# zubair-irshad/NeO-360

Hardware: NVIDIA H100
Metric: rays/sec at 640x480, 192 samples/ray (higher is better)
Workload: dtype f16 operands, f32 accumulate (wgmma)

## Files before the change

### neo360_b200/csrc/field_tc.cu

```cuda
#include "common.cuh"
#include "hopper.cuh"
#include <cuda.h>
#include <cuda_fp16.h>
#include <cstdio>
#include <cstring>

namespace neo {
namespace tc {
using namespace hopper;

constexpr int kTileRays = 32;
constexpr int kTileSamples = 2;
constexpr int kTilePts = kTileRays * kTileSamples;
constexpr int kConsumers = 2;
constexpr int kThreads = 128 * (kConsumers + 1);
constexpr int kLaunchRegs = 65536 / kThreads / 8 * 8;
constexpr int kConsumerRegs = 224, kProducerRegs = 56;
static_assert(kConsumers * 128 * kConsumerRegs + 128 * kProducerRegs == kThreads * kLaunchRegs, "setmaxnreg split must fill the CTA's registers");
static_assert(kConsumers * kTilePts == 128, "the producer warpgroup has one thread per point of each consumer's tile");

constexpr uint32_t WH_H = 0, WH_DIR = 20480, WH_V1 = 30720, WH_RGB = 38912, WH_BYTES = 40960;
constexpr int BIAS_FLOATS = 512 + 64 + 64 + 4 + 4;
constexpr uint32_t BIAS_BYTES = 2624;
constexpr uint32_t SLAB = 128 * 128;

__host__ __device__ constexpr int enc_slabs(int KE) { return (KE + 63) / 64; }
__host__ __device__ constexpr uint32_t trunk_off(int KE, int seg) { return seg == 0 ? 0u : (uint32_t)(enc_slabs(KE) + 2 * (seg - 1)) * SLAB; }
__host__ __device__ constexpr uint32_t trunk_bytes(int KE) { return trunk_off(KE, 4) + (uint32_t)(KE / 64) * SLAB; }
__host__ __device__ constexpr uint32_t w3enc_tail(int KE) { return trunk_off(KE, 0) + (uint32_t)(KE / 64) * SLAB; }
__host__ __device__ constexpr uint32_t w3enc_kstep(int KE, int ks) {
    return ks < 4 * (KE / 64) ? trunk_off(KE, 4) + (uint32_t)(ks >> 2) * SLAB + (uint32_t)(ks & 3) * 32u
                              : w3enc_tail(KE) + (uint32_t)(ks - 4 * (KE / 64) + 2) * 32u;
}

__host__ __device__ inline int pmap_logical(int p) {
    const int q = p & 127, u = q >> 5, t = (q >> 3) & 3, jj = (q >> 1) & 3, e = q & 1;
    return (p & 128) + 8 * (4 * u + jj) + 2 * t + e;
}

struct PtsRow {
    float xe[3];
    float tv;
    float xl[3];
    int rid, sidx;
    int src;
    int valid;
    int pad;
};

struct MlpTc {
    int in_ch, enc_dim, KE;
    const unsigned char* trunkimg;
    const unsigned char* headimg;
    const float* bias;
    const __half* pmap[4];
};

struct State {
    MlpTc mlp[4];
};

struct Params {
    const float *rays_o, *rays_d, *far, *tvals;
    const uint4* dir;
    const int* ray_order;
    int n_rays, N, chunk, nv, n_tiles, sg;
    float far_unc;
    SceneDev sc;
    MlpTc mlp;
    float* rgb_out;
    float* sigma_out;
    int* trap;
#ifdef NEO_FIELD_PHASES
    int phase_slot;
#endif
};

#ifdef NEO_FIELD_PHASES
enum Phase {
    kPhWait, kPhRows, kPhBlend0, kPhLayers, kPhBlend3, kPhLayer3, kPhDir, kPhColour,
    kPhSetup, kPhEnc, kPhTaps, kPhSlot,
    kPhases
};
constexpr int kPhaseCols = kPhases + 3;
constexpr int kPhaseUnits = 2 * kConsumers;
constexpr uint32_t kPhaseBytes = kPhaseUnits * (kPhases + 1) * 8;
constexpr int kPhaseSlots = 64;
__device__ unsigned long long g_phase_cycles[kPhaseSlots][kPhaseCols];
static int g_phase_launches = 0;
#define FIELD_PHASE_INIT(unit, lead) \
    unsigned ph_t = clock();         \
    unsigned long long ph_taps = 0;  \
    unsigned long long ph_shared = 0; \
    const int ph_unit = (unit);      \
    const bool ph_lead = (lead)
#define FIELD_PHASE(p)                                        \
    do {                                                      \
        const unsigned now_ = clock();                        \
        if (ph_lead) ph_acc[ph_unit][p] += now_ - ph_t;       \
        ph_t = now_;                                          \
    } while (0)
#else
constexpr uint32_t kPhaseBytes = 0;
#define FIELD_PHASE_INIT(unit, lead) do {} while (0)
#define FIELD_PHASE(p) do {} while (0)
#endif

__global__ void wsel_kernel(const float* __restrict__ w0, int ld0, int col0, const float* __restrict__ w3, int ld3, int col3, int C, __half* __restrict__ out) {
    const int idx = blockIdx.x * blockDim.x + threadIdx.x;
    if (idx >= 256 * C) return;
    const int r = pmap_logical(idx / C), c = idx % C;
    out[idx] = __float2half_rn(r < 128 ? w0[(size_t)r * ld0 + col0 + c] : w3[(size_t)(r - 128) * ld3 + col3 + c]);
}

struct EncCol { int kind, cc, lvl; };
template <int ICH>
__host__ __device__ constexpr EncCol enc_col(int col) {
    constexpr int STRIDE = (ICH == 3) ? 21 : 24;
    const int cc = col / STRIDE, j = col % STRIDE;
    if (ICH == 3 && col == 63) return {1, 0, 0};
    if (ICH == 4 && col == 21) return {1, 0, 0};
    if (cc >= ICH || j >= 21) return {0, 0, 0};
    if (j == 0) return {2, cc, 0};
    if (j <= 10) return {3, cc, j - 1};
    return {4, cc, j - 11};
}
template <int ICH>
__host__ __device__ constexpr int enc_col_ref_index(int col) {
    const EncCol e = enc_col<ICH>(col);
    if (e.kind == 2) return e.cc;
    if (e.kind == 3) return ICH + e.lvl * ICH + e.cc;
    if (e.kind == 4) return ICH + kPosDeg * ICH + e.lvl * ICH + e.cc;
    return -1;
}
__device__ __forceinline__ uint32_t pack_h2(float a, float b) {
    __half2 h = __floats2half2_rn(a, b);
    return *reinterpret_cast<uint32_t*>(&h);
}
__global__ void trunk_img_kernel(NeoMLPParams p, int enc_dim, int KE, unsigned char* __restrict__ img) {
    const int KW = 2 * KE + 384;
    const int idx = blockIdx.x * blockDim.x + threadIdx.x;
    if (idx >= KW * 128) return;
    const int n = idx / KW, kk = idx % KW;
    const int in_dim = enc_dim + kLocalCh + kWorldCh;
    const bool bg = (KE == 96);
    auto enc_w = [&](const float* w, size_t stride, size_t off0, const float* bias, int col) -> float {
        const EncCol e = bg ? enc_col<4>(col) : enc_col<3>(col);
        if (e.kind == 1) return bias[n];
        const int ref = bg ? enc_col_ref_index<4>(col) : enc_col_ref_index<3>(col);
        return ref >= 0 ? w[(size_t)n * stride + off0 + ref] : 0.f;
    };
    int seg, k;
    float x;
    if (kk < KE) { seg = 0; k = kk; x = enc_w(p.w0, in_dim, 0, p.b0, k); }
    else if (kk < KE + 128) { seg = 1; k = kk - KE; x = p.w1[n * 128 + k]; }
    else if (kk < KE + 256) { seg = 2; k = kk - KE - 128; x = p.w2[n * 128 + k]; }
    else if (kk < KE + 384) { seg = 3; k = kk - KE - 256; x = p.w3[(size_t)n * (128 + in_dim) + k]; }
    else { seg = 4; k = kk - KE - 384; x = enc_w(p.w3, 128 + in_dim, 128, p.b3, k); }
    const int full = 64 * (KE / 64);
    const uint32_t off = (seg == 4 && k >= full) ? w3enc_tail(KE) + sw128_off(n, 32 + k - full, 128) : trunk_off(KE, seg) + sw128_off(n, k, 128);
    *reinterpret_cast<__half*>(img + off) = __float2half_rn(x);
}

__global__ void head_kernel(NeoMLPParams p, int nv, unsigned char* __restrict__ img, float* __restrict__ bias) {
    int idx = blockIdx.x * blockDim.x + threadIdx.x;
    __half* im = reinterpret_cast<__half*>(img);
    const float inv = 1.0f / (float)nv;
    if (idx < 80 * 128) {
        int r = idx / 128, k = idx % 128;
        float x = 0.f;
        if (r < 64) { for (int j = 0; j < 128; ++j) x = fmaf(p.wv0[r * 155 + j], p.wb[j * 128 + k], x); x *= inv; }
        else if (r == 64) x = p.wsig[k] * inv;
        im[(WH_H + sw128_off(r, k, 80)) / 2] = __float2half_rn(x);
    } else if (idx < 80 * 128 + 80 * 64) {
        int e = idx - 80 * 128, r = e / 64, k = e % 64;
        float x = (r < 64 && k < kDirEnc) ? p.wv0[r * 155 + 128 + k] : 0.f;
        im[(WH_DIR + sw128_off(r, k, 80)) / 2] = __float2half_rn(x);
    } else if (idx < 80 * 128 + 80 * 64 + 64 * 64) {
        int e = idx - 80 * 128 - 80 * 64, r = e / 64, k = e % 64;
        im[(WH_V1 + sw128_off(r, k, 64)) / 2] = __float2half_rn(p.wv1[r * 64 + k]);
    } else if (idx < 80 * 128 + 80 * 64 + 64 * 64 + 16 * 64) {
        int e = idx - 80 * 128 - 80 * 64 - 64 * 64, r = e / 64, k = e % 64;
        im[(WH_RGB + sw128_off(r, k, 16)) / 2] = __float2half_rn(r < 3 ? p.wrgb[r * 64 + k] : 0.f);
    }
    if (idx < BIAS_FLOATS) {
        float x = 0.f;
        if (idx < 128) x = p.b0[idx];
        else if (idx < 256) x = p.b1[idx - 128];
        else if (idx < 384) x = p.b2[idx - 256];
        else if (idx < 512) x = p.b3[idx - 384];
        else if (idx < 576) { int r = idx - 512; x = p.bv0[r]; for (int j = 0; j < 128; ++j) x = fmaf(p.wv0[r * 155 + j], p.bb[j], x); }
        else if (idx < 640) x = p.bv1[idx - 576];
        else if (idx < 643) x = p.brgb[idx - 640];
        else if (idx == 644) x = p.bsig[0];
        bias[idx] = x;
    }
}

struct RayFast { float o[3], d[3], far, rho, phi, psph[3], axis[3]; };
__device__ __forceinline__ void ray_fast(const float* __restrict__ o, const float* __restrict__ d, float far, RayFast& g, bool need_bg) {
    g.o[0] = o[0]; g.o[1] = o[1]; g.o[2] = o[2]; g.d[0] = d[0]; g.d[1] = d[1]; g.d[2] = d[2]; g.far = far;
    if (need_bg) {
        const float dd = d[0] * d[0] + d[1] * d[1] + d[2] * d[2];
        const float inv_dd = __fdividef(1.0f, dd);
        const float d1 = -(d[0] * o[0] + d[1] * o[1] + d[2] * o[2]) * inv_dd;
        const float p[3] = {o[0] + d1 * d[0], o[1] + d1 * d[1], o[2] + d1 * d[2]};
        const float p2 = p[0] * p[0] + p[1] * p[1] + p[2] * p[2];
        g.rho = sqrtf(p2);
        const float s = d1 + sqrtf(fmaxf(1.0f - p2, 0.f)) * rsqrtf(dd);
        for (int i = 0; i < 3; ++i) g.psph[i] = o[i] + s * d[i];
        float ax[3] = {o[1] * g.psph[2] - o[2] * g.psph[1], o[2] * g.psph[0] - o[0] * g.psph[2], o[0] * g.psph[1] - o[1] * g.psph[0]};
        const float an = rsqrtf(ax[0] * ax[0] + ax[1] * ax[1] + ax[2] * ax[2]);
        for (int i = 0; i < 3; ++i) g.axis[i] = ax[i] * an;
        g.phi = asinf(g.rho);
    }
}
__device__ __forceinline__ void bg_point_fast(const RayFast& g, float s, float far_unc, float* xhat, float* lin) {
    const float ang = g.phi - asinf(g.rho * s);
    float sa, ca;
    __sincosf(ang, &sa, &ca);
    const float* a = g.axis;
    const float* p = g.psph;
    const float cr[3] = {a[1] * p[2] - a[2] * p[1], a[2] * p[0] - a[0] * p[2], a[0] * p[1] - a[1] * p[0]};
    const float ap = (a[0] * p[0] + a[1] * p[1] + a[2] * p[2]) * (1.0f - ca);
    float q[3];
    for (int i = 0; i < 3; ++i) q[i] = p[i] * ca + cr[i] * sa + a[i] * ap;
    const float qn = __fdividef(1.0f, sqrtf(q[0] * q[0] + q[1] * q[1] + q[2] * q[2]) + 1e-10f);
    for (int i = 0; i < 3; ++i) xhat[i] = q[i] * qn;
    const float tl = g.far * (1.0f - s) + far_unc * s;
    for (int i = 0; i < 3; ++i) lin[i] = g.o[i] + tl * g.d[i];
}

struct TapQuad { int x0, y0; float w[4]; };
__device__ __forceinline__ void tap_quad(float gx, float gy, int W, int H, TapQuad& t) {
    const float ix = ((gx + 1.f) / 2.f) * (float)(W - 1);
    const float iy = ((gy + 1.f) / 2.f) * (float)(H - 1);
    const float x0f = floorf(ix), y0f = floorf(iy);
    const float fx = ix - x0f, fy = iy - y0f;
    const float gx1 = (x0f + 1.f) - ix, gy1 = (y0f + 1.f) - iy;
    const bool inr = (ix >= -1.f) && (ix < (float)W) && (iy >= -1.f) && (iy < (float)H);
    const int x0 = inr ? (int)x0f : -2, y0 = inr ? (int)y0f : -2;
    const bool vx0 = (x0 >= 0) & (x0 < W), vx1 = (x0 + 1 >= 0) & (x0 + 1 < W);
    const bool vy0 = (y0 >= 0) & (y0 < H), vy1 = (y0 + 1 >= 0) & (y0 + 1 < H);
    t.x0 = x0; t.y0 = y0;
    t.w[0] = (inr & vx0 & vy0) ? gx1 * gy1 : 0.f;
    t.w[1] = (inr & vx1 & vy0) ? fx * gy1 : 0.f;
    t.w[2] = (inr & vx0 & vy1) ? gx1 * fy : 0.f;
    t.w[3] = (inr & vx1 & vy1) ? fx * fy : 0.f;
}

enum Chan { kRowsFull, kRowsEmpty, kStageFull, kStageEmpty, kTapsFull, kTapsEmpty, kChans };
constexpr int kBars = 1 + kChans * kConsumers;

__device__ __noinline__ void wait_timeout(int* trapinfo, uint32_t bar, int id) {
    if (trapinfo) {
        volatile int* t = trapinfo;
        if (t[0] == 0) {
            t[1] = (int)blockIdx.x; t[2] = (int)threadIdx.x; t[3] = (int)bar; t[4] = id; t[5] = (int)gridDim.x;
            t[0] = 1000;
        }
        __threadfence_system();
    }
    asm volatile("trap;");
}
__device__ __forceinline__ void bar_wait(int* trapinfo, uint32_t bar0, int id, uint32_t parity) {
    const uint32_t b = bar0 + 8u * (uint32_t)id;
    if (!mbar_wait_bounded(b, parity)) wait_timeout(trapinfo, b, id);
}

__device__ __forceinline__ float sel4(const float* x, int i) { return i == 0 ? x[0] : i == 1 ? x[1] : i == 2 ? x[2] : x[3]; }

constexpr int kStageRow = 64;
__device__ __forceinline__ int stage_slot(int n, int k) { return n * kStageRow + ((((k >> 1) ^ ((n & 7) << 2))) << 1 | (k & 1)); }

__device__ __forceinline__ void stage_items(__half* stage, int n, const float (&x)[3], int first, int count) {
#pragma unroll 1
    for (int i = first; i < first + count; ++i) {
        const int j = i / 10, l = i - 10 * j;
        const float xc = j == 0 ? x[0] : j == 1 ? x[1] : x[2];
        float s, c;
        sincosf(xc * (float)(1 << l), &s, &c);
        stage[stage_slot(n, 21 * j + 1 + l)] = __float2half_rn(s);
        stage[stage_slot(n, 21 * j + 11 + l)] = __float2half_rn(c);
    }
}

template <int ICH>
__device__ __forceinline__ uint32_t enc_staged(const __half* stage, int n, int c0, int u, int j0) {
    if (ICH == 3) {
        const int c = c0 + u;
        return c == 63 ? 0x3c00u : __half_as_ushort(stage[stage_slot(n, c)]);
    }
    const int j = c0 / 24, k = c0 % 24 + u;
    if (k >= 21) return (j == 0 && k == 21) ? 0x3c00u : 0u;
    return __half_as_ushort(stage[stage_slot(n, 21 * (j - j0) + k)]);
}
template <int ICH>
constexpr bool stage_layout_ok() {
    for (int c = 0; c < (ICH == 3 ? 64 : 96); ++c) {
        const EncCol e = enc_col<ICH>(c);
        const int k = e.kind == 2 ? 0 : e.kind == 3 ? 1 + e.lvl : 11 + e.lvl;
        if (ICH == 3 && e.kind >= 2 && c != 21 * e.cc + k) return false;
        if (ICH == 4) {
            const int j = c / 24, kk = c % 24;
            if (e.kind >= 2 && (kk >= 21 || j != e.cc || kk != k)) return false;
            if (e.kind < 2 && kk < 21) return false;
            if ((e.kind == 1) != (j == 0 && kk == 21)) return false;
        }
        if (ICH == 3 && (e.kind == 1) != (c == 63)) return false;
        if (ICH == 3 && e.kind == 0) return false;
    }
    return true;
}
static_assert(stage_layout_ok<3>() && stage_layout_ok<4>(), "enc_staged does not match enc_col");

__device__ __forceinline__ float dir_value(const float* dc, int e) {
    if (e >= kDirEnc) return 0.f;
    if (e < 3) return sel4(dc, e);
    const int q0 = e - 3;
    const bool shifted = q0 >= 12;
    const int qq = shifted ? q0 - 12 : q0;
    const float xb = sel4(dc, qq % 3) * (float)(1 << (qq / 3));
    return sinf(shifted ? xb + 1.57079637f : xb);
}

__device__ __forceinline__ uint4 dir_words(const ViewXform* vxs, int nv, const float (&wd)[3], int t) {
    float dsum[8];
#pragma unroll
    for (int c = 0; c < 8; ++c) dsum[c] = 0.f;
    for (int vv = 0; vv < nv; ++vv) {
        float dc[3];
        rotate_to_camera(vxs[vv], wd, dc);
#pragma unroll
        for (int c = 0; c < 8; ++c) dsum[c] += dir_value(dc, 16 * (c >> 2) + 8 * ((c >> 1) & 1) + 2 * t + (c & 1));
    }
    const float inv = 1.0f / (float)nv;
    return make_uint4(pack_h2(dsum[0] * inv, dsum[1] * inv), pack_h2(dsum[2] * inv, dsum[3] * inv), pack_h2(dsum[4] * inv, dsum[5] * inv),
                      pack_h2(dsum[6] * inv, dsum[7] * inv));
}
__global__ void dir_frag_kernel(const float* __restrict__ viewdirs, int n_rays, const ViewXform* __restrict__ views, int nv, uint4* __restrict__ out) {
    const long long idx = (long long)blockIdx.x * blockDim.x + threadIdx.x;
    if (idx >= 4LL * n_rays) return;
    const long long r = idx >> 2;
    const float wd[3] = {viewdirs[3 * r], viewdirs[3 * r + 1], viewdirs[3 * r + 2]};
    out[idx] = dir_words(views, nv, wd, (int)(idx & 3));
}

template <int NC>
__device__ __forceinline__ void relu_to_frags(const float (&d)[NC / 2], uint32_t (&a)[NC / 16][4]) {
#pragma unroll
    for (int ks = 0; ks < NC / 16; ++ks)
#pragma unroll
        for (int r = 0; r < 4; ++r) a[ks][r] = pack_h2(fmaxf(d[8 * ks + 2 * r], 0.f), fmaxf(d[8 * ks + 2 * r + 1], 0.f));
}
template <int NC>
__device__ __forceinline__ void seed_bias(float (&d)[NC / 2], const float* b, int t) {
#pragma unroll
    for (int j = 0; j < NC / 8; ++j)
#pragma unroll
        for (int i = 0; i < 2; ++i) { d[4 * j + 2 * i] = b[8 * j + 2 * t]; d[4 * j + 2 * i + 1] = b[8 * j + 2 * t + 1]; }
}
__device__ __forceinline__ uint64_t wdesc(uint32_t base, int ks, uint32_t slab) { return desc_sw128(base + (uint32_t)(ks >> 2) * slab + (uint32_t)(ks & 3) * 32u); }

struct TapTable {
    int4 tex[4][kTilePts];
    float4 w[4][kTilePts];
    uint16_t share[kTilePts / 2];
};
__host__ __device__ constexpr int share_pair(int r0) { return (r0 >> 4) * 8 + (r0 & 7); }
__device__ __forceinline__ int comp4(const int4& x, int k) { return k == 0 ? x.x : k == 1 ? x.y : k == 2 ? x.z : x.w; }
__device__ __forceinline__ float comp4(const float4& x, int k) { return k == 0 ? x.x : k == 1 ? x.y : k == 2 ? x.z : x.w; }

template <bool SHARE>
__device__ __forceinline__ uint32_t tap_entry(TapTable& tab, const SceneDev& sc, const float (&cl)[3], int v, int n, int m) {
    float gx, gy;
    int mw, mh;
    if (m == 0) {
        local_grid_coords(sc, cl, gx, gy);
        mw = sc.lat_w; mh = sc.lat_h;
    } else {
        gx = (m == 3) ? cl[1] : cl[0];
        gy = (m == 2) ? cl[1] : cl[2];
        mw = sc.plane_w; mh = sc.plane_h;
    }
    TapQuad tq;
    tap_quad(gx, gy, mw, mh, tq);
    int tx[4];
#pragma unroll
    for (int k = 0; k < 4; ++k) tx[k] = tq.w[k] == 0.f ? 0 : (v * mh + tq.y0 + (k >> 1)) * mw + tq.x0 + (k & 1);
    tab.tex[m][n] = make_int4(tx[0], tx[1], tx[2], tx[3]);
    tab.w[m][n] = make_float4(tq.w[0], tq.w[1], tq.w[2], tq.w[3]);
    if (!SHARE) return 0;
    uint32_t shared = 0;
#pragma unroll
    for (int k = 0; k < 4; ++k) {
        const int key = tq.w[k] == 0.f ? -1 : tx[k];
        const int other = __shfl_down_sync(0xffffffffu, key, 8);
        shared |= (uint32_t)(key >= 0 && key == other) << k;
    }
    return shared;
}

template <int I>
__device__ __forceinline__ void blend_tap(float (&acc)[64], float w, const uint4 (&q)[4]) {
#pragma unroll
    for (int u = 0; u < 4; ++u) {
        const uint32_t wd[4] = {q[u].x, q[u].y, q[u].z, q[u].w};
#pragma unroll
        for (int jj = 0; jj < 4; ++jj) {
            const float2 f = __half22float2(*reinterpret_cast<const __half2*>(&wd[jj]));
            const int j = 4 * u + jj;
            acc[4 * j + 2 * I] = fmaf(w, f.x, acc[4 * j + 2 * I]);
            acc[4 * j + 2 * I + 1] = fmaf(w, f.y, acc[4 * j + 2 * I + 1]);
        }
    }
}

template <int HALF, bool PAIR>
__device__ __forceinline__ void blend_maps(float (&acc)[64], const Params& P, const TapTable& tab, int r0, int t) {
    uint32_t share = PAIR ? tab.share[share_pair(r0)] : 0u;
#pragma unroll 1
    for (int m = 0; m < 4; ++m, share >>= 4) {
        const float4 wv0 = tab.w[m][r0], wv1 = tab.w[m][r0 + 8];
        const int* tx0 = reinterpret_cast<const int*>(&tab.tex[m][r0]);
        const int* tx1 = reinterpret_cast<const int*>(&tab.tex[m][r0 + 8]);
        const uint4* base = reinterpret_cast<const uint4*>(P.mlp.pmap[m] + HALF * 128 + t * 8);
#pragma unroll
        for (int k = 0; k < 4; ++k) {
            const float w0 = comp4(wv0, k), w1 = comp4(wv1, k);
            const bool both = (share >> k) & 1u;
            uint4 q0[4], q1[4];
            if (w0 != 0.f) {
#pragma unroll
                for (int u = 0; u < 4; ++u) q0[u] = __ldg(base + (size_t)tx0[k] * 32 + 4 * u);
                if (!PAIR) blend_tap<0>(acc, w0, q0);
            }
            if (w1 != 0.f && !both)
#pragma unroll
                for (int u = 0; u < 4; ++u) q1[u] = __ldg(base + (size_t)tx1[k] * 32 + 4 * u);
            if (PAIR && w0 != 0.f) blend_tap<0>(acc, w0, q0);
            if (w1 != 0.f) {
                if (both)
#pragma unroll
                    for (int u = 0; u < 4; ++u) q1[u] = q0[u];
                blend_tap<1>(acc, w1, q1);
            }
        }
    }
}

template <int KE>
struct SmemMap {
    static constexpr uint32_t HEAD = trunk_bytes(KE), BIAS = HEAD + WH_BYTES, VIEWS = BIAS + BIAS_BYTES,
                              PTS = VIEWS + kMaxViews * 64, TAPS = PTS + kConsumers * kTilePts * (uint32_t)sizeof(PtsRow),
                              STAGE = TAPS + kConsumers * (uint32_t)sizeof(TapTable),
                              BAR = STAGE + kConsumers * kTilePts * kStageRow * (uint32_t)sizeof(__half),
                              PHASES = BAR + (kBars * 8 + 15) / 16 * 16, TOTAL = PHASES + kPhaseBytes;
    static_assert(KE % 64 == 0 || KE % 64 == 32, "an encoding segment ends on a whole or a half slab (w3enc_tail)");
    static_assert(TOTAL + 1024 <= 227u * 1024u, "field kernel shared memory exceeds the 227 KB an sm_90 CTA can have");
};

template <int ICH>
__global__ void __launch_bounds__(kThreads, 1) field_tc_kernel(const __grid_constant__ Params P) {
    extern __shared__ __align__(1024) unsigned char smem_raw[];
    const uint32_t sbase = (smem_u32(smem_raw) + 1023u) & ~1023u;
    unsigned char* sgen = smem_raw + (sbase - smem_u32(smem_raw));
    constexpr int KE = (ICH == 3) ? 64 : 96, KS = KE / 16;
    constexpr bool IS_BG = (ICH == 4);
    using SM = SmemMap<KE>;
    const uint32_t bar = sbase + SM::BAR;

    if (threadIdx.x == 0) {
        mbar_init(bar, 1);
        for (int c = 0; c < kConsumers; ++c)
            for (int k = 0; k < kChans; ++k) mbar_init(bar + 8u * (1 + kChans * c + k), (k & 1) ? 128 : kTilePts);
        mbar_init_fence();
        constexpr uint32_t TB = trunk_bytes(KE);
        mbar_expect_tx(bar, TB + WH_BYTES + BIAS_FLOATS * 4);
        for (uint32_t off = 0; off < TB; off += 32768u) bulk_load(sbase + off, P.mlp.trunkimg + off, min(32768u, TB - off), bar);
        bulk_load(sbase + SM::HEAD, P.mlp.headimg, WH_BYTES, bar);
        bulk_load(sbase + SM::BIAS, P.mlp.bias, BIAS_FLOATS * 4, bar);
    }
    {
        float* vsm = reinterpret_cast<float*>(sgen + SM::VIEWS);
        const float* vsrc = reinterpret_cast<const float*>(P.sc.views);
        for (int i = threadIdx.x; i < P.nv * 16; i += kThreads) vsm[i] = __ldg(vsrc + i);
    }
#ifdef NEO_FIELD_PHASES
    auto ph_acc = reinterpret_cast<unsigned long long (*)[kPhases + 1]>(sgen + SM::PHASES);
    if (threadIdx.x < kPhaseUnits * (kPhases + 1)) (&ph_acc[0][0])[threadIdx.x] = 0ull;
#endif
    __syncthreads();

    const int wg = threadIdx.x >> 7;
    const ViewXform* vxs = reinterpret_cast<const ViewXform*>(sgen + SM::VIEWS);
    const int nv = P.nv, N = P.N;

    if (wg == kConsumers) {
        setmaxnreg_dec<kProducerRegs>();
        const int pt = threadIdx.x - 128 * kConsumers, c = pt / kTilePts, n = pt % kTilePts;
        PtsRow* pts = reinterpret_cast<PtsRow*>(sgen + SM::PTS) + c * kTilePts;
        TapTable* tab = reinterpret_cast<TapTable*>(sgen + SM::TAPS) + c;
        __half* stage = reinterpret_cast<__half*>(sgen + SM::STAGE) + c * kTilePts * kStageRow;
        const int cb = 1 + kChans * c;
        uint32_t k_rows = 0, k_stage = 0, k_taps = 0;
        FIELD_PHASE_INIT(kConsumers + c, n == 0);
        for (int tile = blockIdx.x * kConsumers + c; tile < P.n_tiles; tile += gridDim.x * kConsumers) {
            const int g = tile / P.sg, q = tile % P.sg;
            bar_wait(P.trap, bar, cb + kRowsEmpty, (k_rows & 1) ^ 1);
            FIELD_PHASE(kPhSlot);
            {
                const int rl = n % kTileRays, sl = n / kTileRays;
                const int slot = g * kTileRays + rl, s = q * kTileSamples + sl;
                const int slot_c = min(slot, P.n_rays - 1), s_c = min(s, N - 1);
                const int rid = P.ray_order ? P.ray_order[slot_c] : slot_c;
                PtsRow pr;
                pr.rid = rid; pr.sidx = s_c; pr.valid = (slot < P.n_rays) && (s < N);
                pr.tv = P.tvals[(long long)rid * N + s_c];
                RayFast rg;
                ray_fast(P.rays_o + 3 * rid, P.rays_d + 3 * rid, P.far[rid], rg, IS_BG);
                if (IS_BG) bg_point_fast(rg, pr.tv, P.far_unc, pr.xe, pr.xl);
                else for (int i = 0; i < 3; ++i) { pr.xe[i] = rg.o[i] + pr.tv * rg.d[i]; pr.xl[i] = pr.xe[i]; }
                const int ch = P.chunk > 0 ? P.chunk : P.n_rays;
                const int c0 = (rid / ch) * ch;
                const int Bc = min(ch, P.n_rays - c0);
                const long long jl = (long long)(rid - c0) * N + s_c;
                pr.src = c0 + (int)(jl % Bc);
                pr.pad = 0;
                pts[n] = pr;
            }
            mbar_arrive(bar + 8u * (cb + kRowsFull));
            ++k_rows;
            FIELD_PHASE(kPhSetup);
            if constexpr (IS_BG) {
                const float sx[3] = {pts[n].tv, 0.f, 0.f};
                bar_wait(P.trap, bar, cb + kStageEmpty, (k_stage & 1) ^ 1);
                FIELD_PHASE(kPhSlot);
                stage[stage_slot(n, 0)] = __float2half_rn(sx[0]);
                stage_items(stage, n, sx, 0, 10);
                mbar_arrive(bar + 8u * (cb + kStageFull));
                ++k_stage;
                FIELD_PHASE(kPhEnc);
            }
#pragma unroll 1
            for (int v = 0; v < nv; ++v) {
                float ce[3];
                to_camera(vxs[v], pts[n].xe, ce);
                bar_wait(P.trap, bar, cb + kStageEmpty, (k_stage & 1) ^ 1);
                FIELD_PHASE(kPhSlot);
#pragma unroll
                for (int j = 0; j < 3; ++j) stage[stage_slot(n, 21 * j)] = __float2half_rn(ce[j]);
                stage_items(stage, n, ce, 0, 30);
                mbar_arrive(bar + 8u * (cb + kStageFull));
                ++k_stage;
                FIELD_PHASE(kPhEnc);
                float cl[3] = {ce[0], ce[1], ce[2]};
                if constexpr (IS_BG) to_camera(vxs[v], pts[n].xl, cl);
                bar_wait(P.trap, bar, cb + kTapsEmpty, (k_taps & 1) ^ 1);
                FIELD_PHASE(kPhSlot);
                uint32_t shared = 0;
#pragma unroll 1
                for (int m = 0; m < 4; ++m) {
                    shared |= tap_entry<!IS_BG>(*tab, P.sc, cl, v, n, m) << (4 * m);
#ifdef NEO_FIELD_PHASES
                    for (int k = 0; k < 4; ++k) ph_taps += comp4(tab->w[m][n], k) != 0.f;
#endif
                }
                if (!IS_BG && (n & 15) < 8) {
                    tab->share[share_pair(n)] = (uint16_t)shared;
#ifdef NEO_FIELD_PHASES
                    ph_shared += __popc(shared);
#endif
                }
                mbar_arrive(bar + 8u * (cb + kTapsFull));
                ++k_taps;
                FIELD_PHASE(kPhTaps);
            }
        }
#ifdef NEO_FIELD_PHASES
        if (ph_lead)
            for (int p = kPhSetup; p < kPhases; ++p) atomicAdd(&g_phase_cycles[P.phase_slot][p], ph_acc[ph_unit][p]);
        atomicAdd(&g_phase_cycles[P.phase_slot][kPhases + 1], ph_taps);
        atomicAdd(&g_phase_cycles[P.phase_slot][kPhases + 2], ph_shared);
#endif
        return;
    }

    setmaxnreg_inc<kConsumerRegs>();
    bar_wait(P.trap, bar, 0, 0);
    const int wt = threadIdx.x & 127, warp = wt >> 5, lane = threadIdx.x & 31, t = lane & 3;
    const PtsRow* pts = reinterpret_cast<const PtsRow*>(sgen + SM::PTS) + wg * kTilePts;
    const TapTable* tab = reinterpret_cast<const TapTable*>(sgen + SM::TAPS) + wg;
    const __half* stage = reinterpret_cast<const __half*>(sgen + SM::STAGE) + wg * kTilePts * kStageRow;
    const int cb = 1 + kChans * wg;
    uint32_t k_rows = 0, k_stage = 0, k_taps = 0;
    const float* sb = reinterpret_cast<const float*>(sgen + SM::BIAS);
    const uint32_t sW = sbase, sH = sbase + SM::HEAD;
    const int r0 = warp * 16 + (lane >> 2);
    FIELD_PHASE_INIT(wg, wt == 0);

    for (int tile = blockIdx.x * kConsumers + wg; tile < P.n_tiles; tile += gridDim.x * kConsumers) {
        bar_wait(P.trap, bar, cb + kRowsFull, k_rows & 1);
        FIELD_PHASE(kPhWait);
        long long gp[2];
        int src[2];
#pragma unroll
        for (int i = 0; i < 2; ++i) {
            const PtsRow& pr = pts[r0 + 8 * i];
            gp[i] = pr.valid ? (long long)pr.rid * N + pr.sidx : -1;
            src[i] = pr.src;
        }
        mbar_arrive(bar + 8u * (cb + kRowsEmpty));
        ++k_rows;
#ifdef NEO_FIELD_PHASES
        if (wt == 0) ph_acc[wg][kPhases] += 1ull;
#endif
        uint32_t enc[KS][4];
        auto load_enc = [&](int ks, int h, int j0) {
#pragma unroll
            for (int i = 0; i < 2; ++i)
                enc[ks][2 * h + i] = enc_staged<ICH>(stage, r0 + 8 * i, 16 * ks + 8 * h, 2 * t, j0) |
                                     enc_staged<ICH>(stage, r0 + 8 * i, 16 * ks + 8 * h, 2 * t + 1, j0) << 16;
        };
        if constexpr (IS_BG) {
            bar_wait(P.trap, bar, cb + kStageFull, k_stage & 1);
            FIELD_PHASE(kPhWait);
            load_enc(KS - 2, 1, 3);
            load_enc(KS - 1, 0, 3);
            load_enc(KS - 1, 1, 3);
            mbar_arrive(bar + 8u * (cb + kStageEmpty));
            ++k_stage;
        }
        FIELD_PHASE(kPhRows);

        float hacc[40];
#pragma unroll
        for (int i = 0; i < 40; ++i) hacc[i] = 0.f;
#pragma unroll 1
        for (int v = 0; v < nv; ++v) {
            bar_wait(P.trap, bar, cb + kStageFull, k_stage & 1);
            FIELD_PHASE(kPhWait);
#pragma unroll
            for (int ks = 0; ks < 4; ++ks)
#pragma unroll
                for (int h = 0; h < 2; ++h) load_enc(ks, h, 0);
            if constexpr (IS_BG) load_enc(4, 0, 0);
            mbar_arrive(bar + 8u * (cb + kStageEmpty));
            ++k_stage;
            FIELD_PHASE(kPhRows);
            bar_wait(P.trap, bar, cb + kTapsFull, k_taps & 1);
            FIELD_PHASE(kPhWait);
            float acc[64];
            uint32_t a[8][4];
#pragma unroll
            for (int i = 0; i < 64; ++i) acc[i] = 0.f;
            blend_maps<0, !IS_BG>(acc, P, *tab, r0, t);
            FIELD_PHASE(kPhBlend0);
            wgmma_fence();
#pragma unroll
            for (int ks = 0; ks < KS; ++ks) wgmma_rs_n128(acc, enc[ks], wdesc(sW + trunk_off(KE, 0), ks, SLAB));
            wgmma_commit();
            wgmma_wait<0>();
            relu_to_frags<128>(acc, a);
#pragma unroll 1
            for (int l = 1; l <= 2; ++l) {
                seed_bias<128>(acc, sb + 128 * l, t);
                wgmma_fence();
#pragma unroll
                for (int ks = 0; ks < 8; ++ks) wgmma_rs_n128(acc, a[ks], wdesc(sW + trunk_off(KE, l), ks, SLAB));
                wgmma_commit();
                wgmma_wait<0>();
                relu_to_frags<128>(acc, a);
            }
#pragma unroll
            for (int i = 0; i < 64; ++i) acc[i] = 0.f;
            FIELD_PHASE(kPhLayers);
            blend_maps<1, !IS_BG>(acc, P, *tab, r0, t);
            mbar_arrive(bar + 8u * (cb + kTapsEmpty));
            ++k_taps;
            FIELD_PHASE(kPhBlend3);
            wgmma_fence();
#pragma unroll
            for (int ks = 0; ks < 8; ++ks) wgmma_rs_n128(acc, a[ks], wdesc(sW + trunk_off(KE, 3), ks, SLAB));
#pragma unroll
            for (int ks = 0; ks < KS; ++ks) wgmma_rs_n128(acc, enc[ks], desc_sw128(sW + w3enc_kstep(KE, ks)));
            wgmma_commit();
            wgmma_wait<0>();
            relu_to_frags<128>(acc, a);
            wgmma_fence();
#pragma unroll
            for (int ks = 0; ks < 8; ++ks) wgmma_rs_n80(hacc, a[ks], wdesc(sH + WH_H, ks, 80 * 128));
            wgmma_commit();
            wgmma_wait<0>();
            FIELD_PHASE(kPhLayer3);
        }
        {
            const uint4 d0 = __ldg(P.dir + 4LL * src[0] + t), d1 = __ldg(P.dir + 4LL * src[1] + t);
            const uint32_t dfr[2][4] = {{d0.x, d1.x, d0.y, d1.y}, {d0.z, d1.z, d0.w, d1.w}};
            wgmma_fence();
#pragma unroll
            for (int ks = 0; ks < 2; ++ks) wgmma_rs_n80(hacc, dfr[ks], wdesc(sH + WH_DIR, ks, 80 * 128));
            wgmma_commit();
            wgmma_wait<0>();
        }
        FIELD_PHASE(kPhDir);
        if (t == 0) {
#pragma unroll
            for (int i = 0; i < 2; ++i) {
                const float xs = (hacc[32 + 2 * i] + sb[644]) - 1.0f;
                if (gp[i] >= 0) P.sigma_out[gp[i]] = softplus_(xs);
            }
        }
        uint32_t qa[4][4];
#pragma unroll
        for (int ks = 0; ks < 4; ++ks)
#pragma unroll
            for (int r = 0; r < 4; ++r) {
                const int c = 16 * ks + 8 * (r >> 1) + 2 * t;
                qa[ks][r] = pack_h2(fmaxf(hacc[8 * ks + 2 * r] + sb[512 + c], 0.f), fmaxf(hacc[8 * ks + 2 * r + 1] + sb[512 + c + 1], 0.f));
            }
        float v1[32];
        seed_bias<64>(v1, sb + 576, t);
        wgmma_fence();
#pragma unroll
        for (int ks = 0; ks < 4; ++ks) wgmma_rs_n64(v1, qa[ks], wdesc(sH + WH_V1, ks, 64 * 128));
        wgmma_commit();
        wgmma_wait<0>();
        relu_to_frags<64>(v1, qa);
        float o[8];
#pragma unroll
        for (int j = 0; j < 2; ++j)
#pragma unroll
            for (int i = 0; i < 2; ++i)
#pragma unroll
                for (int e = 0; e < 2; ++e) {
                    const int c = 8 * j + 2 * t + e;
                    o[4 * j + 2 * i + e] = c < 3 ? sb[640 + c] : 0.f;
                }
        wgmma_fence();
#pragma unroll
        for (int ks = 0; ks < 4; ++ks) wgmma_rs_n16(o, qa[ks], wdesc(sH + WH_RGB, ks, 16 * 128));
        wgmma_commit();
        wgmma_wait<0>();
        if (t < 2) {
#pragma unroll
            for (int i = 0; i < 2; ++i) {
                if (gp[i] < 0) continue;
#pragma unroll
                for (int e = 0; e < 2; ++e) {
                    const int c = 2 * t + e;
                    if (c < 3) P.rgb_out[gp[i] * 3 + c] = rgb_act(o[2 * i + e]);
                }
            }
        }
        FIELD_PHASE(kPhColour);
    }
#ifdef NEO_FIELD_PHASES
    if (ph_lead) {
        for (int p = 0; p < kPhSetup; ++p) atomicAdd(&g_phase_cycles[P.phase_slot][p], ph_acc[ph_unit][p]);
        atomicAdd(&g_phase_cycles[P.phase_slot][kPhases], ph_acc[ph_unit][kPhases]);
    }
#endif
}

}

static int* g_trap_host = nullptr;
static int* g_trap_dev = nullptr;

static int trap_buffer() {
    if (g_trap_host) return NEO_OK;
    void* h = nullptr;
    NEO_CUDA(cudaHostAlloc(&h, 8 * sizeof(int), cudaHostAllocMapped));
    memset(h, 0, 8 * sizeof(int));
    void* dptr = nullptr;
    NEO_CUDA(cudaHostGetDevicePointer(&dptr, h, 0));
    g_trap_host = (int*)h;
    g_trap_dev = (int*)dptr;
    return NEO_OK;
}
const char* tc_trap_info() {
    static char buf[256];
    if (!g_trap_host || g_trap_host[0] == 0) return "";
    volatile int* t = g_trap_host;
    static const char* chans[tc::kChans] = {"rows full", "rows empty", "staging full", "staging empty", "tap table full", "tap table empty"};
    const int id = t[4];
    char what[64];
    if (id == 0) snprintf(what, sizeof(what), "weight copies");
    else if (id > 0 && id < tc::kBars) snprintf(what, sizeof(what), "%s, consumer %d", chans[(id - 1) % tc::kChans], (id - 1) / tc::kChans);
    else snprintf(what, sizeof(what), "barrier %d", id);
    snprintf(buf, sizeof(buf), " [TC field kernel: wait on the %s mbarrier timed out: CTA %d of %d, thread %d, barrier smem 0x%x]",
             what, t[1], t[5], t[2], (unsigned)t[3]);
    return buf;
}

int tc_scene_create(NeoScene* sc, const NeoMLPParams mlps[4], cudaStream_t s) {
    using namespace tc;
    const NeoSceneDesc& d = sc->desc;
    State* st = new State();
    sc->tc_state = st;
    const float* planes[3] = {d.planes_xz, d.planes_xy, d.planes_yz};
    struct Temps {
        __half* feat16[4] = {nullptr, nullptr, nullptr, nullptr};
        size_t bytes[4] = {0, 0, 0, 0};
        __half* wsel = nullptr;
        cudaStream_t s;
        ~Temps() {
            cudaStreamSynchronize(s);
            for (int k = 0; k < 4; ++k) pool_release(feat16[k], bytes[k]);
            pool_release(wsel, (size_t)256 * kLocalCh * 2);
        }
    } tmp;
    tmp.s = s;
    if ((long long)d.nv * d.lat_h * d.lat_w > 0x7fffffffLL || (long long)d.nv * d.plane_h * d.plane_w > 0x7fffffffLL) {
        set_error("feature maps too large: the tap table holds 32-bit texel indices");
        return NEO_ERR_UNSUPPORTED;
    }
    __half** feat16 = tmp.feat16;
    __half*& wsel = tmp.wsel;
    {
        const float* srcs[4] = {d.latent, planes[0], planes[1], planes[2]};
        int rc;
        for (int k = 0; k < 4; ++k) {
            const int C = k ? kWorldCh : kLocalCh, hw = k ? d.plane_h * d.plane_w : d.lat_h * d.lat_w;
            tmp.bytes[k] = (size_t)d.nv * hw * C * 2;
            if ((rc = pool_alloc((void**)&feat16[k], tmp.bytes[k]))) return rc;
            if ((rc = launch_nchw_to_nhwc(srcs[k], feat16[k], d.nv, C, hw, s))) return rc;
        }
        if ((rc = pool_alloc((void**)&wsel, (size_t)256 * kLocalCh * 2))) return rc;
    }
    for (int i = 0; i < 4; ++i) {
        const NeoMLPParams& p = mlps[i];
        if (p.in_ch != 3 && p.in_ch != 4) { set_error("mlp %d: in_ch must be 3 or 4", i); return NEO_ERR_INVALID; }
        if ((i & 1) != (p.in_ch == 4)) { set_error("mlps must be ordered fg_coarse, bg_coarse, fg_fine, bg_fine"); return NEO_ERR_INVALID; }
        MlpTc& m = st->mlp[i];
        m.in_ch = p.in_ch;
        m.enc_dim = p.in_ch * 21;
        m.KE = (p.in_ch == 3) ? 64 : 96;
        const int in_dim = m.enc_dim + kLocalCh + kWorldCh;
        void* q = nullptr;
        int rc;
        const uint32_t tbytes = trunk_bytes(m.KE);
        if ((rc = scene_alloc_bytes(sc, &q, tbytes))) return rc;
        m.trunkimg = (const unsigned char*)q;
        const int nelem = (2 * m.KE + 384) * 128;
        trunk_img_kernel<<<(nelem + 255) / 256, 256, 0, s>>>(p, m.enc_dim, m.KE, (unsigned char*)q);
        NEO_LAUNCH_CHECK("trunk_img_kernel");
        void* hb = nullptr; void* bb = nullptr;
        if ((rc = scene_alloc_bytes(sc, &hb, WH_BYTES))) return rc;
        if ((rc = scene_alloc_bytes(sc, &bb, BIAS_BYTES))) return rc;
        NEO_CUDA(cudaMemsetAsync(hb, 0, WH_BYTES, s));
        NEO_CUDA(cudaMemsetAsync(bb, 0, BIAS_BYTES, s));
        head_kernel<<<(80 * 128 + 80 * 64 + 64 * 64 + 16 * 64 + 255) / 256, 256, 0, s>>>(p, d.nv, (unsigned char*)hb, (float*)bb);
        NEO_LAUNCH_CHECK("head_kernel");
        m.headimg = (const unsigned char*)hb;
        m.bias = (const float*)bb;
        for (int k = 0; k < 4; ++k) {
            const int C = k ? kWorldCh : kLocalCh, mh = k ? d.plane_h : d.lat_h, mw = k ? d.plane_w : d.lat_w, hw = mh * mw;
            const int col = m.enc_dim + (k ? kLocalCh : 0);
            void* pp = nullptr;
            if ((rc = scene_alloc_bytes(sc, &pp, (size_t)d.nv * hw * 256 * 2))) return rc;
            m.pmap[k] = (const __half*)pp;
            wsel_kernel<<<(256 * C + 255) / 256, 256, 0, s>>>(p.w0, in_dim, col, p.w3, 128 + in_dim, 128 + col, C, wsel);
            NEO_LAUNCH_CHECK("wsel_kernel");
            for (int v = 0; v < d.nv; ++v)
                if ((rc = gemm_f16(feat16[k] + (size_t)v * hw * C, C, wsel, C, nullptr, (__half*)pp + (size_t)v * hw * 256, 256, hw, 256, C, 0, s)))
                    return rc;
        }
        NEO_CUDA(cudaStreamSynchronize(s));
    }
    NEO_CUDA(cudaStreamSynchronize(s));
    return NEO_OK;
}

void tc_scene_free(NeoScene* sc) {
    if (sc && sc->tc_state) { delete reinterpret_cast<tc::State*>(sc->tc_state); sc->tc_state = nullptr; }
}

int launch_dir_frags(const NeoScene* sc, const NeoRays* rays, void* dir, cudaStream_t s) {
    if (!rays->viewdirs || !dir || (uintptr_t)dir % 16) { set_error("direction fragments: need viewdirs and a 16-byte aligned output"); return NEO_ERR_INVALID; }
    const long long threads = 4LL * rays->n_rays;
    if (threads <= 0) return NEO_OK;
    tc::dir_frag_kernel<<<(unsigned)((threads + 255) / 256), 256, 0, s>>>(rays->viewdirs, rays->n_rays, sc->dev.views, sc->dev.nv,
                                                                         static_cast<uint4*>(dir));
    NEO_LAUNCH_CHECK("dir_frag_kernel");
    return NEO_OK;
}

int launch_field_tc(const NeoScene* sc, const NeoRays* rays, const float* far, const float* t, int N, int mlp_index, const void* dir,
                    float* rgb, float* sigma, cudaStream_t s) {
    using namespace tc;
    if (!(sc->precision_mask & (1 << NEO_PREC_TC)) || !sc->tc_state) { set_error("scene was not prepared for NEO_PREC_TC"); return NEO_ERR_INVALID; }
    if (!dir) { set_error("NEO_PREC_TC field launch without direction fragments"); return NEO_ERR_INVALID; }
    const State* st = reinterpret_cast<const State*>(sc->tc_state);
    static int n_sm_of[64] = {0};
    int dev = 0;
    NEO_CUDA(cudaGetDevice(&dev));
    if (dev < 0 || dev >= 64) { set_error("device index %d out of range", dev); return NEO_ERR_UNSUPPORTED; }
    if (!n_sm_of[dev]) NEO_CUDA(cudaDeviceGetAttribute(&n_sm_of[dev], cudaDevAttrMultiProcessorCount, dev));
    const int n_sm = n_sm_of[dev];
    Params P;
    P.rays_o = rays->rays_o; P.rays_d = rays->rays_d; P.far = far; P.tvals = t;
    P.dir = static_cast<const uint4*>(dir);
    P.ray_order = rays->ray_order;
    P.n_rays = rays->n_rays; P.N = N; P.chunk = rays->chunk; P.nv = sc->dev.nv;
    P.sg = (N + kTileSamples - 1) / kTileSamples;
    const long long groups = ((long long)rays->n_rays + kTileRays - 1) / kTileRays;
    const long long n_tiles = groups * P.sg;
    if (n_tiles > 0x3fffffffLL) { set_error("too many tiles"); return NEO_ERR_UNSUPPORTED; }
    P.n_tiles = (int)n_tiles;
    P.far_unc = 3.0f;
    P.sc = sc->dev;
    P.mlp = st->mlp[mlp_index];
    P.rgb_out = rgb; P.sigma_out = sigma;
    { int rc0 = trap_buffer(); if (rc0) return rc0; }
    P.trap = g_trap_dev;
#ifdef NEO_FIELD_PHASES
    P.phase_slot = g_phase_launches++ % kPhaseSlots;
#endif
    const long long ctas = (n_tiles + kConsumers - 1) / kConsumers;
    const int grid = (int)(ctas < n_sm ? ctas : n_sm);
    auto launch = [&](auto kern, size_t smem) -> int {
        cudaFuncAttributes fa;
        NEO_CUDA(cudaFuncGetAttributes(&fa, kern));
        if (fa.numRegs != kLaunchRegs) {
            set_error("field_tc_kernel was compiled for %d registers per thread, its warpgroup split needs %d", fa.numRegs, kLaunchRegs);
            return NEO_ERR_UNSUPPORTED;
        }
        NEO_CUDA(cudaFuncSetAttribute(kern, cudaFuncAttributeMaxDynamicSharedMemorySize, (int)smem));
        kern<<<grid, kThreads, smem, s>>>(P);
        return NEO_OK;
    };
    int rc;
    if (mlp_index & 1) rc = launch(field_tc_kernel<4>, SmemMap<96>::TOTAL + 1024);
    else rc = launch(field_tc_kernel<3>, SmemMap<64>::TOTAL + 1024);
    if (rc != NEO_OK) return rc;
    NEO_LAUNCH_CHECK("field_tc_kernel");
    return NEO_OK;
}

}

extern "C" int neo_tc_enc_column(int in_ch, int col) {
    using namespace neo::tc;
    if ((in_ch != 3 && in_ch != 4) || col < 0 || col >= (in_ch == 3 ? 64 : 96)) return -3;
    const EncCol e = (in_ch == 3) ? enc_col<3>(col) : enc_col<4>(col);
    if (e.kind == 1) return -1;
    if (e.kind == 0) return -2;
    return (in_ch == 3) ? enc_col_ref_index<3>(col) : enc_col_ref_index<4>(col);
}
extern "C" const char* neo_tc_trap_info(void) { return neo::tc_trap_info(); }

#ifdef NEO_FIELD_PHASES
extern "C" int neo_field_phases_reset(void) {
    neo::tc::g_phase_launches = 0;
    void* p = nullptr;
    if (cudaGetSymbolAddress(&p, neo::tc::g_phase_cycles) != cudaSuccess) return -1;
    return cudaMemset(p, 0, sizeof(neo::tc::g_phase_cycles)) == cudaSuccess ? 0 : -1;
}
extern "C" int neo_field_phases_read(unsigned long long* out, int max_launches) {
    using namespace neo::tc;
    if (g_phase_launches > kPhaseSlots) return -1;
    const int n = g_phase_launches < max_launches ? g_phase_launches : max_launches;
    if (n > 0 && cudaMemcpyFromSymbol(out, g_phase_cycles, sizeof(unsigned long long) * n * kPhaseCols) != cudaSuccess) return -1;
    return n;
}
#endif
```

Baseline: 664,000.

## Stage background time encoding with point rows and compact tap table to base indices

For the background field, the per-tile time-encoding columns are now written by the producer into a dedicated bank-conflict-free row buffer alongside the point rows. This removes an extra stage-buffer handshake (full/empty barrier round trip) per tile, and consumers read the words straight from that buffer. The tap table also stores one base texel index per map instead of four indices, and the other three are recomputed from the map width at blend time. That cuts shared-memory footprint and store traffic in exchange for a little integer arithmetic per tap.

```diff
diff --git a/neo360_b200/csrc/field_tc.cu b/neo360_b200/csrc/field_tc.cu
--- a/neo360_b200/csrc/field_tc.cu
+++ b/neo360_b200/csrc/field_tc.cu
@@ -273,27 +273,28 @@
 constexpr int kStageRow = 64;
 __device__ __forceinline__ int stage_slot(int n, int k) { return n * kStageRow + ((((k >> 1) ^ ((n & 7) << 2))) << 1 | (k & 1)); }
 
-__device__ __forceinline__ void stage_items(__half* stage, int n, const float (&x)[3], int first, int count) {
+template <typename Slot>
+__device__ __forceinline__ void stage_items(__half* rows, Slot slot, const float (&x)[3], int first, int count) {
 #pragma unroll 1
     for (int i = first; i < first + count; ++i) {
         const int j = i / 10, l = i - 10 * j;
         const float xc = j == 0 ? x[0] : j == 1 ? x[1] : x[2];
         float s, c;
         sincosf(xc * (float)(1 << l), &s, &c);
-        stage[stage_slot(n, 21 * j + 1 + l)] = __float2half_rn(s);
-        stage[stage_slot(n, 21 * j + 11 + l)] = __float2half_rn(c);
+        rows[slot(21 * j + 1 + l)] = __float2half_rn(s);
+        rows[slot(21 * j + 11 + l)] = __float2half_rn(c);
     }
 }
 
 template <int ICH>
-__device__ __forceinline__ uint32_t enc_staged(const __half* stage, int n, int c0, int u, int j0) {
+__device__ __forceinline__ uint32_t enc_staged(const __half* stage, int n, int c0, int u) {
     if (ICH == 3) {
         const int c = c0 + u;
         return c == 63 ? 0x3c00u : __half_as_ushort(stage[stage_slot(n, c)]);
     }
     const int j = c0 / 24, k = c0 % 24 + u;
     if (k >= 21) return (j == 0 && k == 21) ? 0x3c00u : 0u;
-    return __half_as_ushort(stage[stage_slot(n, 21 * (j - j0) + k)]);
+    return __half_as_ushort(stage[stage_slot(n, 21 * j + k)]);
 }
 template <int ICH>
 constexpr bool stage_layout_ok() {
@@ -314,6 +315,29 @@
 }
 static_assert(stage_layout_ok<3>() && stage_layout_ok<4>(), "enc_staged does not match enc_col");
 
+constexpr int kSRow = 24;
+constexpr int kSCol0 = 72;
+__device__ __forceinline__ uint32_t s_word(const __half* srows, int n, int k) {
+    return *reinterpret_cast<const uint32_t*>(srows + n * kSRow + k);
+}
+constexpr bool s_layout_ok() {
+    for (int k = 0; k < kSRow; ++k) {
+        const EncCol e = enc_col<4>(kSCol0 + k);
+        const int slot = e.kind == 2 ? 0 : e.kind == 3 ? 1 + e.lvl : 11 + e.lvl;
+        if (k < 21 && (e.kind < 2 || e.cc != 3 || slot != k)) return false;
+        if (k >= 21 && e.kind != 0) return false;
+    }
+    if (kSCol0 + kSRow != 96 || kSRow % 2) return false;
+    for (int h = 0; h < 3; ++h) {
+        unsigned banks = 0;
+        for (int r = 0; r < 8; ++r)
+            for (int t = 0; t < 4; ++t) banks |= 1u << ((r * kSRow + 8 * h + 2 * t) / 2 % 32);
+        if (banks != 0xffffffffu) return false;
+    }
+    return true;
+}
+static_assert(s_layout_ok(), "s rows do not match enc_col<4> or their fragment loads conflict on banks");
+
 __device__ __forceinline__ float dir_value(const float* dc, int e) {
     if (e >= kDirEnc) return 0.f;
     if (e < 3) return sel4(dc, e);
@@ -363,13 +387,13 @@
 __device__ __forceinline__ uint64_t wdesc(uint32_t base, int ks, uint32_t slab) { return desc_sw128(base + (uint32_t)(ks >> 2) * slab + (uint32_t)(ks & 3) * 32u); }
 
 struct TapTable {
-    int4 tex[4][kTilePts];
+    int base[4][kTilePts];
     float4 w[4][kTilePts];
     uint16_t share[kTilePts / 2];
 };
 __host__ __device__ constexpr int share_pair(int r0) { return (r0 >> 4) * 8 + (r0 & 7); }
-__device__ __forceinline__ int comp4(const int4& x, int k) { return k == 0 ? x.x : k == 1 ? x.y : k == 2 ? x.z : x.w; }
 __device__ __forceinline__ float comp4(const float4& x, int k) { return k == 0 ? x.x : k == 1 ? x.y : k == 2 ? x.z : x.w; }
+__device__ __forceinline__ int tap_index(int base, int mw, int k) { return base + (k >> 1) * mw + (k & 1); }
 
 template <bool SHARE>
 __device__ __forceinline__ uint32_t tap_entry(TapTable& tab, const SceneDev& sc, const float (&cl)[3], int v, int n, int m) {
@@ -388,7 +412,8 @@
     int tx[4];
 #pragma unroll
     for (int k = 0; k < 4; ++k) tx[k] = tq.w[k] == 0.f ? 0 : (v * mh + tq.y0 + (k >> 1)) * mw + tq.x0 + (k & 1);
-    tab.tex[m][n] = make_int4(tx[0], tx[1], tx[2], tx[3]);
+    const bool any = (tq.w[0] != 0.f) | (tq.w[1] != 0.f) | (tq.w[2] != 0.f) | (tq.w[3] != 0.f);
+    tab.base[m][n] = any ? (v * mh + tq.y0) * mw + tq.x0 : 0;
     tab.w[m][n] = make_float4(tq.w[0], tq.w[1], tq.w[2], tq.w[3]);
     if (!SHARE) return 0;
     uint32_t shared = 0;
@@ -416,14 +441,16 @@
     }
 }
 
-template <int HALF, bool PAIR>
+template <int HALF, bool PAIR, bool SHARE>
 __device__ __forceinline__ void blend_maps(float (&acc)[64], const Params& P, const TapTable& tab, int r0, int t) {
-    uint32_t share = PAIR ? tab.share[share_pair(r0)] : 0u;
+    static_assert(PAIR || !SHARE, "a shared tap is blended into both rows from one load: the paired form");
+    uint32_t share = SHARE ? tab.share[share_pair(r0)] : 0u;
 #pragma unroll 1
     for (int m = 0; m < 4; ++m, share >>= 4) {
         const float4 wv0 = tab.w[m][r0], wv1 = tab.w[m][r0 + 8];
-        const int* tx0 = reinterpret_cast<const int*>(&tab.tex[m][r0]);
-        const int* tx1 = reinterpret_cast<const int*>(&tab.tex[m][r0 + 8]);
+        const int* bx0 = &tab.base[m][r0];
+        const int* bx1 = &tab.base[m][r0 + 8];
+        const int mw = m == 0 ? P.sc.lat_w : P.sc.plane_w;
         const uint4* base = reinterpret_cast<const uint4*>(P.mlp.pmap[m] + HALF * 128 + t * 8);
 #pragma unroll
         for (int k = 0; k < 4; ++k) {
@@ -431,13 +458,16 @@
             const bool both = (share >> k) & 1u;
             uint4 q0[4], q1[4];
             if (w0 != 0.f) {
-#pragma unroll
-                for (int u = 0; u < 4; ++u) q0[u] = __ldg(base + (size_t)tx0[k] * 32 + 4 * u);
+                const int tx = tap_index(*bx0, mw, k);
+#pragma unroll
+                for (int u = 0; u < 4; ++u) q0[u] = __ldg(base + (size_t)tx * 32 + 4 * u);
                 if (!PAIR) blend_tap<0>(acc, w0, q0);
             }
-            if (w1 != 0.f && !both)
-#pragma unroll
-                for (int u = 0; u < 4; ++u) q1[u] = __ldg(base + (size_t)tx1[k] * 32 + 4 * u);
+            if (w1 != 0.f && !both) {
+                const int tx = tap_index(*bx1, mw, k);
+#pragma unroll
+                for (int u = 0; u < 4; ++u) q1[u] = __ldg(base + (size_t)tx * 32 + 4 * u);
+            }
             if (PAIR && w0 != 0.f) blend_tap<0>(acc, w0, q0);
             if (w1 != 0.f) {
                 if (both)
@@ -454,7 +484,8 @@
     static constexpr uint32_t HEAD = trunk_bytes(KE), BIAS = HEAD + WH_BYTES, VIEWS = BIAS + BIAS_BYTES,
                               PTS = VIEWS + kMaxViews * 64, TAPS = PTS + kConsumers * kTilePts * (uint32_t)sizeof(PtsRow),
                               STAGE = TAPS + kConsumers * (uint32_t)sizeof(TapTable),
-                              BAR = STAGE + kConsumers * kTilePts * kStageRow * (uint32_t)sizeof(__half),
+                              SROWS = STAGE + kConsumers * kTilePts * kStageRow * (uint32_t)sizeof(__half),
+                              BAR = SROWS + (KE == 96 ? kConsumers * kTilePts * kSRow * (uint32_t)sizeof(__half) : 0u),
                               PHASES = BAR + (kBars * 8 + 15) / 16 * 16, TOTAL = PHASES + kPhaseBytes;
     static_assert(KE % 64 == 0 || KE % 64 == 32, "an encoding segment ends on a whole or a half slab (w3enc_tail)");
     static_assert(TOTAL + 1024 <= 227u * 1024u, "field kernel shared memory exceeds the 227 KB an sm_90 CTA can have");
@@ -502,6 +533,7 @@
         PtsRow* pts = reinterpret_cast<PtsRow*>(sgen + SM::PTS) + c * kTilePts;
         TapTable* tab = reinterpret_cast<TapTable*>(sgen + SM::TAPS) + c;
         __half* stage = reinterpret_cast<__half*>(sgen + SM::STAGE) + c * kTilePts * kStageRow;
+        __half* srows = reinterpret_cast<__half*>(sgen + SM::SROWS) + c * kTilePts * kSRow;
         const int cb = 1 + kChans * c;
         uint32_t k_rows = 0, k_stage = 0, k_taps = 0;
         FIELD_PHASE_INIT(kConsumers + c, n == 0);
@@ -528,20 +560,18 @@
                 pr.src = c0 + (int)(jl % Bc);
                 pr.pad = 0;
                 pts[n] = pr;
+                if constexpr (IS_BG) {
+                    const float sx[3] = {pr.tv, 0.f, 0.f};
+                    __half* srow = srows + n * kSRow;
+                    srow[0] = __float2half_rn(sx[0]);
+                    stage_items(srow, [](int k) { return k; }, sx, 0, 10);
+#pragma unroll
+                    for (int k = 21; k < kSRow; ++k) srow[k] = __float2half_rn(0.f);
+                }
             }
             mbar_arrive(bar + 8u * (cb + kRowsFull));
             ++k_rows;
             FIELD_PHASE(kPhSetup);
-            if constexpr (IS_BG) {
-                const float sx[3] = {pts[n].tv, 0.f, 0.f};
-                bar_wait(P.trap, bar, cb + kStageEmpty, (k_stage & 1) ^ 1);
-                FIELD_PHASE(kPhSlot);
-                stage[stage_slot(n, 0)] = __float2half_rn(sx[0]);
-                stage_items(stage, n, sx, 0, 10);
-                mbar_arrive(bar + 8u * (cb + kStageFull));
-                ++k_stage;
-                FIELD_PHASE(kPhEnc);
-            }
 #pragma unroll 1
             for (int v = 0; v < nv; ++v) {
                 float ce[3];
@@ -550,7 +580,7 @@
                 FIELD_PHASE(kPhSlot);
 #pragma unroll
                 for (int j = 0; j < 3; ++j) stage[stage_slot(n, 21 * j)] = __float2half_rn(ce[j]);
-                stage_items(stage, n, ce, 0, 30);
+                stage_items(stage, [n](int k) { return stage_slot(n, k); }, ce, 0, 30);
                 mbar_arrive(bar + 8u * (cb + kStageFull));
                 ++k_stage;
                 FIELD_PHASE(kPhEnc);
@@ -592,6 +622,7 @@
     const PtsRow* pts = reinterpret_cast<const PtsRow*>(sgen + SM::PTS) + wg * kTilePts;
     const TapTable* tab = reinterpret_cast<const TapTable*>(sgen + SM::TAPS) + wg;
     const __half* stage = reinterpret_cast<const __half*>(sgen + SM::STAGE) + wg * kTilePts * kStageRow;
+    const __half* srows = reinterpret_cast<const __half*>(sgen + SM::SROWS) + wg * kTilePts * kSRow;
     const int cb = 1 + kChans * wg;
     uint32_t k_rows = 0, k_stage = 0, k_taps = 0;
     const float* sb = reinterpret_cast<const float*>(sgen + SM::BIAS);
@@ -604,33 +635,29 @@
         FIELD_PHASE(kPhWait);
         long long gp[2];
         int src[2];
+        uint32_t enc[KS][4];
 #pragma unroll
         for (int i = 0; i < 2; ++i) {
             const PtsRow& pr = pts[r0 + 8 * i];
             gp[i] = pr.valid ? (long long)pr.rid * N + pr.sidx : -1;
             src[i] = pr.src;
+            if constexpr (IS_BG) {
+                enc[KS - 2][2 + i] = s_word(srows, r0 + 8 * i, 2 * t);
+                enc[KS - 1][i] = s_word(srows, r0 + 8 * i, 8 + 2 * t);
+                enc[KS - 1][2 + i] = s_word(srows, r0 + 8 * i, 16 + 2 * t);
+            }
         }
         mbar_arrive(bar + 8u * (cb + kRowsEmpty));
         ++k_rows;
 #ifdef NEO_FIELD_PHASES
         if (wt == 0) ph_acc[wg][kPhases] += 1ull;
 #endif
-        uint32_t enc[KS][4];
-        auto load_enc = [&](int ks, int h, int j0) {
+        auto load_enc = [&](int ks, int h) {
 #pragma unroll
             for (int i = 0; i < 2; ++i)
-                enc[ks][2 * h + i] = enc_staged<ICH>(stage, r0 + 8 * i, 16 * ks + 8 * h, 2 * t, j0) |
-                                     enc_staged<ICH>(stage, r0 + 8 * i, 16 * ks + 8 * h, 2 * t + 1, j0) << 16;
+                enc[ks][2 * h + i] = enc_staged<ICH>(stage, r0 + 8 * i, 16 * ks + 8 * h, 2 * t) |
+                                     enc_staged<ICH>(stage, r0 + 8 * i, 16 * ks + 8 * h, 2 * t + 1) << 16;
         };
-        if constexpr (IS_BG) {
-            bar_wait(P.trap, bar, cb + kStageFull, k_stage & 1);
-            FIELD_PHASE(kPhWait);
-            load_enc(KS - 2, 1, 3);
-            load_enc(KS - 1, 0, 3);
-            load_enc(KS - 1, 1, 3);
-            mbar_arrive(bar + 8u * (cb + kStageEmpty));
-            ++k_stage;
-        }
         FIELD_PHASE(kPhRows);
 
         float hacc[40];
@@ -643,8 +670,8 @@
 #pragma unroll
             for (int ks = 0; ks < 4; ++ks)
 #pragma unroll
-                for (int h = 0; h < 2; ++h) load_enc(ks, h, 0);
-            if constexpr (IS_BG) load_enc(4, 0, 0);
+                for (int h = 0; h < 2; ++h) load_enc(ks, h);
+            if constexpr (IS_BG) load_enc(4, 0);
             mbar_arrive(bar + 8u * (cb + kStageEmpty));
             ++k_stage;
             FIELD_PHASE(kPhRows);
@@ -654,7 +681,7 @@
             uint32_t a[8][4];
 #pragma unroll
             for (int i = 0; i < 64; ++i) acc[i] = 0.f;
-            blend_maps<0, !IS_BG>(acc, P, *tab, r0, t);
+            blend_maps<0, !IS_BG, !IS_BG>(acc, P, *tab, r0, t);
             FIELD_PHASE(kPhBlend0);
             wgmma_fence();
 #pragma unroll
@@ -675,7 +702,7 @@
 #pragma unroll
             for (int i = 0; i < 64; ++i) acc[i] = 0.f;
             FIELD_PHASE(kPhLayers);
-            blend_maps<1, !IS_BG>(acc, P, *tab, r0, t);
+            blend_maps<1, !IS_BG, !IS_BG>(acc, P, *tab, r0, t);
             mbar_arrive(bar + 8u * (cb + kTapsEmpty));
             ++k_taps;
             FIELD_PHASE(kPhBlend3);
```

After: 684,300, median of 6. 1.03x the previous value.
